# MeryylleA/Lunaris-Orion

Measured on AMD Instinct MI355X. Metric: 128x128 sprites/sec, VAE training step (train_hybrid.py _process_batch), latent_dim=512, higher is better.
Workload: dtype f16; 1 GPU; VAE-only training step (fwd+MSE/KL+bwd+clip+AdamW), per-GPU batch 64, latent_dim 512, teacher scalar 0 (--reward_scale 0 --quality_weight 0; the full hybrid step of BASELINE config 3 is the config3_full_hybrid object of a --full run at N=1), gradient_accumulation_steps 1, fp16 MFMA operands / fp32 accumulate, fp32 master weights; global_batch=64, latent_dim=512, parallelism=single, linear_weight_gradients=factored (never materialised)

## Files before the change

### lunaris_orion_amd/csrc/lo_conv.h

```cpp
#pragma once
#include "lo_common.h"

int lo_pack_weight(const float* w, f16* wp, const LoGeom& g, hipStream_t st);
int lo_pack_all(const LoPackJob* jobs_dev, int njobs, int nblocks, hipStream_t st, int block_base = 0);
int lo_pack_blocks(const LoGeom& g);
size_t lo_packed_weight_elems(const LoGeom& g);
static inline int lo_geom_packed_elems(const LoGeom& g) {
  int off = 0;
  for (int p = 0; p < g.n_phase; ++p) off += g.Cout * g.T[p] * g.Cin;
  return off;
}
static inline double lo_geom_flops(const LoGeom& g) {
  double f = 0;
  for (int p = 0; p < g.n_phase; ++p) f += 2.0 * g.B * g.GH * g.GW * (double)g.Cout * g.T[p] * g.Cin;
  return f;
}
static inline double lo_geom_bytes(const LoGeom& g) {
  return 2.0 * ((double)g.B * g.Hin * g.Win * g.Cin + (double)g.B * g.Hout * g.Wout * g.Cout + lo_geom_packed_elems(g));
}

struct LoGnBwdFuse {
  const f16* v; const float* stats; const float* gamma; const float* beta; float* P1;
  f16* dv = nullptr; float* P2 = nullptr; unsigned int* counter = nullptr; unsigned int target = 0; unsigned int* fail = nullptr;
  bool keep_out = false;
// ... 56 lines not shown
int lo_conv3_run(const LoGeom& g, const LoConvOp& op, const LoConvChoice& c, hipStream_t st);
int lo_convt4_patch_run(const LoGeom& g, const LoConvOp& op, const LoConvChoice& c, hipStream_t st);
int lo_convs2d_patch_run(const LoGeom& g, const LoConvOp& op, const LoConvChoice& c, hipStream_t st);
bool lo_conv3_pp_applies(const LoGeom& g);
bool lo_conv3_pp_f8_applies(const LoGeom& g);
int lo_conv3_pp_rows(const LoGeom& g);
int lo_conv3_run_pp_xf(const LoGeom& g, const f16* in, const f16* xc, const f16* kx, int nlev, const f16* wp, const float* bias,
                       f16* out, hipStream_t st, const LoConvExtra* ex);
int lo_conv3_run_pp_f8(const LoGeom& g, const uint8_t* in8, const uint8_t* w8, const float* wscale, const float* bias, f16* out,
                       hipStream_t st, const LoConvExtra* ex);

struct LoPackF8Job { const f16* src; uint8_t* dst; float* scale; int K[LO_MAX_PHASE]; int wofs[LO_MAX_PHASE]; int Cout, n_phase, block0; };
void lo_pack_f8_job(LoPackF8Job* j, const LoGeom& g, const f16* src, uint8_t* dst, float* scale, int block0);
int lo_pack_f8_all(const LoPackF8Job* jobs_dev, int njobs, int nblocks, hipStream_t st, int block_base = 0);
int lo_pack_f8_one(const LoGeom& g, const f16* wp, uint8_t* w8, float* wscale, hipStream_t st);
int lo_quantize_f8(const f16* x, uint8_t* x8, size_t n, hipStream_t st);

enum LoWgradKernel { LO_WK_WGRAD3 = 0, LO_WK_WGRAD2, LO_WK_TN };
enum LoWgradReduce { LO_WR_NONE = 0, LO_WR_ROWS, LO_WR_CONVT, LO_WR_SCATTER };
struct LoWgradChoice {
  int kernel;
  int bmw, bnw, bkp, stages;
  int taps;
  int tw;
  bool convt;
  int tiles;
  int units, units_per_split;
  int nsplit;
  int slabs;
  dim3 grid, block;
  bool direct;
  int reduce;
  dim3 rgrid, rblock;
};
LoWgradChoice lo_wgrad_choose(const LoGeom& g);
int lo_wgrad_run(const LoGeom& g, const f16* x, const f16* dy, float* slab, float* grad, float scale, hipStream_t st);
size_t lo_wgrad_slab_bytes(const LoGeom& g);
int lo_wgrad3_run(const LoGeom& g, const LoWgradChoice& p, const f16* x, const f16* dy, float* slab, hipStream_t st);
int lo_wgrad2_run(const LoGeom& g, const LoWgradChoice& p, const f16* x, const f16* dy, float* slab, hipStream_t st);
```

### lunaris_orion_amd/csrc/lo_norm.hip

```cpp
#include "lo_norm.h"
#include <stdlib.h>
#include <type_traits>

#define GN_EPS 1e-5f

enum { GN_MODE_PLAIN = 0, GN_MODE_SKIP = 1, GN_MODE_RES = 2 };

int lo_gn_nchunk(int HW, int C) {
  constexpr long chunk_elems = 16384;
  const long ce = (long)HW * C >= 524288 ? 2 * chunk_elems : chunk_elems;
  long e = (long)HW * C / ce;
  if (e < 1) e = 1;
  if (e > 256) e = 256;
  while (HW % e) --e;
  return (int)e;
}

struct GnFwdArgs {
  const f16* v;
  const float* partial;
  const float* gamma;
  const float* beta;
  const f16* other;
  f16* y;
// ... 399 lines not shown
  for (int c = tid; c < G; c += 256) {
    const int ccx = c >> 3, j = c & 7;
    float tot = 0.f;
    for (int sl = 0; sl < nslot; ++sl) tot += s_red[(sl * CG + ccx) * 8 + j];
    a.P2[(size_t)n * C + grp * G + c] = tot;
  }
}

__global__ __launch_bounds__(256) void lo_gn_param_finalize_kernel(const float* __restrict__ P1, const float* __restrict__ P2,
                                                                   float* dgamma, float* dbeta, float* dbias, int nblk, int C,
                                                                   float scale) {
  __shared__ float red[3][16][17];
  const int cl = threadIdx.x & 15, r = threadIdx.x >> 4;
  const int c = blockIdx.x * 16 + cl;
  float g1 = 0.f, g2 = 0.f, b = 0.f;
  if (c < C)
    for (int k = r; k < nblk; k += 16) {
      f32x2 p = *reinterpret_cast<const f32x2*>(P1 + ((size_t)k * C + c) * 2);
      g1 += p[0];
      g2 += p[1];
      b += P2[(size_t)k * C + c];
    }
  red[0][r][cl] = g1; red[1][r][cl] = g2; red[2][r][cl] = b;
  __syncthreads();
  if (r < 3 && c < C) {
    float tot = 0.f;
#pragma unroll
    for (int q = 0; q < 16; ++q) tot += red[r][q][cl];
    tot *= scale;
    if (r == 0) dbeta[c] = tot; else if (r == 1) dgamma[c] = tot; else dbias[c] = tot;
  }
}

__global__ __launch_bounds__(256) void lo_gn_finalize_all_kernel(LoGnFinJobs jobs, float scale) {
  __shared__ float red[3][64][5];
  int jb = 0;
  while (jb + 1 < jobs.n && (int)blockIdx.x >= jobs.j[jb + 1].block0) ++jb;
  const LoGnFinJob& J = jobs.j[jb];
  const int C = J.C;
  const int cl = threadIdx.x & 3, r = threadIdx.x >> 2;
  const int c = ((int)blockIdx.x - J.block0) * 4 + cl;
  float g1 = 0.f, g2 = 0.f, b = 0.f;
  if (c < C) {
    for (int k = r; k < J.nblk1; k += 64) {
      f32x2 p = *reinterpret_cast<const f32x2*>(J.P1 + ((size_t)k * C + c) * 2);
      g1 += p[0];
      g2 += p[1];
    }
    for (int k = r; k < J.nblk2; k += 64) b += J.P2[(size_t)k * C + c];
  }
  red[0][r][cl] = g1; red[1][r][cl] = g2; red[2][r][cl] = b;
  __syncthreads();
  if (threadIdx.x < 12) {
    const int which = threadIdx.x >> 2, c2 = threadIdx.x & 3;
    const int cg = ((int)blockIdx.x - J.block0) * 4 + c2;
    if (cg < C) {
      float tot = 0.f;
      for (int q = 0; q < 64; ++q) tot += red[which][q][c2];
      tot *= scale;
      if (which == 0) J.dbeta[cg] = tot; else if (which == 1) J.dgamma[cg] = tot; else J.dbias[cg] = tot;
    }
  }
}

__global__ __launch_bounds__(256) void lo_transpose_tile_kernel(const f16* __restrict__ src, f16* __restrict__ dst, uint8_t* __restrict__ dst8,
                                                                int R, int Cc) {
  __shared__ f16 tile[64][66];
  const int n = blockIdx.z, r0 = blockIdx.y * 64, c0 = blockIdx.x * 64;
  const f16* s = src + (size_t)n * R * Cc;
  const int tc = (threadIdx.x & 7) * 8, tr = threadIdx.x >> 3;
#pragma unroll
  for (int p = 0; p < 2; ++p) {
    const int r = tr + 32 * p;
    const f16x8 v = *reinterpret_cast<const f16x8*>(s + (size_t)(r0 + r) * Cc + c0 + tc);
#pragma unroll
    for (int j = 0; j < 8; ++j) tile[r][tc + j] = v[j];
  }
  __syncthreads();
  f16* d = dst + (size_t)n * R * Cc;
#pragma unroll
  for (int p = 0; p < 2; ++p) {
    const int c = tr + 32 * p;
    f16x8 v;
#pragma unroll
    for (int j = 0; j < 8; ++j) v[j] = tile[tc + j][c];
    const size_t off = (size_t)(c0 + c) * R + r0 + tc;
    *reinterpret_cast<f16x8*>(d + off) = v;
    if (dst8) {
// ... 175 lines not shown
    return LO_OK;
  }
  if (ch.form == LO_GNB_LOCAL) {
    LoProfScope _p(gn_layer_name("lo_gn_bwd_local", C, HW, mode), 0, 2.0 * B * HW * C * (mode == 2 ? 5 : 3), st);
    gn_launch_local(a, GnSlabSrc{nullptr, 0, nullptr, nullptr, 0}, B, st);
    LO_LAUNCH_CHECK("gn_bwd_local");
    return LO_OK;
  }
  LO_REQUIRE(C % 32 == 0 && C <= 512, "lo_gn_bwd: C=%d unsupported", C);
  if (ch.form == LO_GNB_TWO_PASS) {
    LoProfScope _p(gn_layer_name("lo_gn_bwd_reduce", C, HW, mode), 0, 2.0 * B * HW * C * (mode == 2 ? 4 : 2), st);
    gn_launch_reduce(a, B, st);
  }
  LO_LAUNCH_CHECK("gn_bwd_reduce");
  {
    LoProfScope _p(gn_layer_name("lo_gn_bwd_apply", C, HW, mode), 0, 2.0 * B * HW * C * (mode == 2 ? 4 : 3), st);
    gn_launch_apply(a, B, st);
  }
  LO_LAUNCH_CHECK("gn_bwd_apply");
  return LO_OK;
}

int lo_gn_bwd(const LoGnLayer& l, const LoGnBwd& op, float* dgamma, float* dbeta, float* dbias, float scale, hipStream_t st) {
  LoGnRows rows;
  int r = lo_gn_backward(l, op, st, &rows);
  if (r != LO_OK) return r;
  LoProfScope _p3("lo_gn_param_finalize", 0, 0, st);
  hipLaunchKernelGGL(lo_gn_param_finalize_kernel, dim3((l.C + 15) / 16), dim3(256), 0, st, op.P1, op.P2, dgamma, dbeta, dbias,
                     l.B * rows.p1, l.C, scale);
  LO_LAUNCH_CHECK("gn_param_finalize");
  return LO_OK;
}

int lo_gn_finalize_all(const LoGnFinJobs& jobs, float scale, hipStream_t st) {
  int nblocks = 0;
  for (int i = 0; i < jobs.n; ++i) nblocks += (jobs.j[i].C + 3) / 4;
  LoProfScope _p("lo_gn_finalize_all", 0, 0, st);
  hipLaunchKernelGGL(lo_gn_finalize_all_kernel, dim3(nblocks), dim3(256), 0, st, jobs, scale);
  LO_LAUNCH_CHECK("gn_finalize_all");
  return LO_OK;
}

int lo_nhwc_to_nchw_f16(const f16* src, f16* dst, int B, int HW, int C, hipStream_t st) {
  LO_REQUIRE(HW % 64 == 0 && C % 64 == 0, "lo_nhwc_to_nchw_f16: HW=%d, C=%d must be multiples of 64", HW, C);
  LoProfScope _p("lo_layout_transpose", 0, 4.0 * B * HW * C, st);
  LO_LAUNCH_STOP(lo_transpose_tile_kernel, dim3(C / 64, HW / 64, B), dim3(256), 0, st, src, dst, (uint8_t*)nullptr, HW, C);
  LO_LAUNCH_CHECK("nhwc_to_nchw");
  return LO_OK;
}
int lo_nchw_to_nhwc_f16(const f16* src, f16* dst, int B, int HW, int C, hipStream_t st, uint8_t* dst8) {
  LO_REQUIRE(HW % 64 == 0 && C % 64 == 0, "lo_nchw_to_nhwc_f16: HW=%d, C=%d must be multiples of 64", HW, C);
  LoProfScope _p("lo_layout_transpose", 0, 4.0 * B * HW * C, st);
  LO_LAUNCH_STOP(lo_transpose_tile_kernel, dim3(HW / 64, C / 64, B), dim3(256), 0, st, src, dst, dst8, C, HW);
  LO_LAUNCH_CHECK("nchw_to_nhwc");
  return LO_OK;
}

template <typename TI, typename TO>
__global__ __launch_bounds__(256) void lo_transpose_convert_kernel(const TI* __restrict__ src, TO* __restrict__ dst, int R, int Cc, float scale) {
  __shared__ float tile[64][65];
  const int n = blockIdx.z, r0 = blockIdx.y * 64, c0 = blockIdx.x * 64;
  const TI* s = src + (size_t)n * R * Cc;
  const int tc = threadIdx.x & 63, tr = threadIdx.x >> 6;
#pragma unroll
  for (int p = 0; p < 16; ++p) tile[tr + 4 * p][tc] = (float)s[(size_t)(r0 + tr + 4 * p) * Cc + c0 + tc] * scale;
  __syncthreads();
  TO* d = dst + (size_t)n * R * Cc;
#pragma unroll
  for (int p = 0; p < 16; ++p) d[(size_t)(c0 + tr + 4 * p) * R + r0 + tc] = (TO)tile[tc][tr + 4 * p];
// ... 14 lines not shown
```

### lunaris_orion_amd/csrc/lo_vae_plan.hip

```cpp
#include "lo_vae.h"
#include <memory>

namespace {
struct Arena {
  size_t off = 0;
  size_t take(size_t bytes) {
    size_t o = off;
    off += (bytes + 255) & ~(size_t)255;
    return o;
  }
};
bool env_is_zero(const char* v) { return v && atoi(v) == 0; }
const int kEncCh[5] = {3, 64, 128, 256, 512};
const int kDecCh[5] = {512, 256, 128, 64, 32};
}

static bool layer_takes_f8(const LoGeom& gf) {
  if (lo_conv_choose(gf, {.bias = true, .gn_partial = true, .f8 = true}).kernel == LO_CK_NONE) return false;
  return lo_conv_choose(gf, {.bias = true, .gn_partial = true}).kernel != LO_CK_CONVT4_PATCH;
}

static int setup_conv_layer(ConvLayer& c, int kind, int B, int H, int W, int Cin, int Cout, int p_w, Arena& ar, bool first, bool fp8_fwd) {
  c.kind = kind; c.H = H; c.W = W; c.Cin = Cin; c.Cout = Cout;
  c.p_w = p_w; c.p_b = p_w + 1; c.p_gw = p_w + 2; c.p_gb = p_w + 3;
// ... 292 lines not shown
  const float sc = h->fac.scale / (float)world;
  LO_TRY(lo_lowrank_materialize_gathered(G + h->p_off[h->idx_fc_mu_w], vae_fac_in_block(h, base, h->o_fac_xT), vae_fac_in_block(h, base, h->o_fac_dmlT),
                                         blk, world, 2 * L, 32768, h->B, sc, st));
  return lo_lowrank_materialize_gathered(G + h->p_off[h->idx_dfc_w], vae_fac_in_block(h, base, h->o_fac_zT), vae_fac_in_block(h, base, h->o_fac_gfcT),
                                         blk, world, 32768, L, h->B, sc, st);
}
extern "C" int lo_vae_linear_factored(const LoVae* h) { return h ? vae_flat_lacks_linear(h) : 0; }
extern "C" int lo_vae_num_params(const LoVae* h) { return h->nparam; }
extern "C" size_t lo_vae_param_offset(const LoVae* h, int i) { return (i >= 0 && i < h->nparam) ? h->p_off[i] : (size_t)-1; }
extern "C" size_t lo_vae_param_numel(const LoVae* h, int i) { return (i >= 0 && i < h->nparam) ? h->p_numel[i] : 0; }
extern "C" size_t lo_vae_flat_elems(const LoVae* h) { return h->flat_elems; }
extern "C" size_t lo_vae_workspace_bytes(const LoVae* h) { return h->ws_bytes; }

extern "C" int lo_vae_debug_tensor(const LoVae* h, int which, int s, int k, size_t* byte_offset, int* dims4) {
  LO_REQUIRE(h && byte_offset && dims4 && s >= 0 && s < 4 && k >= 0 && k < 3, "lo_vae_debug_tensor: bad argument");
  const ConvLayer* c = which == 0 ? &h->enc[s][k] : ((which == 1 || which == 3) ? &h->dec[s] : (which == 2 ? &h->enc[s][2] : nullptr));
  LO_REQUIRE(c, "lo_vae_debug_tensor: unknown tensor kind %d", which);
  *byte_offset = which == 2 ? h->o_eout[s] : (which == 3 ? c->o_a : c->o_v);
  dims4[0] = h->B; dims4[1] = c->Ho; dims4[2] = c->Wo; dims4[3] = c->Cout;
  return LO_OK;
}

extern "C" int lo_vae_debug_tensor_ex(const LoVae* h, int which, int s, int k, size_t* byte_offset, int* dims4, int* elem_bytes) {
  LO_REQUIRE(h && byte_offset && dims4 && elem_bytes && s >= 0 && s < 4 && k >= 0 && k < 3, "lo_vae_debug_tensor_ex: bad argument");
  *elem_bytes = 2;
  if (which >= 0 && which <= 3) return lo_vae_debug_tensor(h, which, s, k, byte_offset, dims4);
  dims4[0] = h->B;
  if (which == 9) { *byte_offset = h->o_h0; dims4[1] = dims4[2] = 8; dims4[3] = 512; return LO_OK; }
  if (which == 10) {
    LO_REQUIRE(s < 3, "lo_vae_debug_tensor_ex: three skip gradients, asked for %d", s);
    *byte_offset = h->o_skipg[s]; dims4[1] = dims4[2] = 64 >> s; dims4[3] = 64 << s;
    return LO_OK;
  }
  LO_REQUIRE(which >= 4 && which <= 8 && !(which == 4 && k == 2), "lo_vae_debug_tensor_ex: unknown tensor kind %d (k = %d)", which, k);
  const ConvLayer* c = (which == 6 || which == 8) ? &h->dec[s] : &h->enc[s][k];
  if (which == 5 || which == 6) {
    *byte_offset = c->o_stats; *elem_bytes = 4;
    dims4[1] = 8; dims4[2] = 2; dims4[3] = 1;
    return LO_OK;
  }
  *byte_offset = which == 4 ? c->o_a : ((c == &h->enc[0][0] && !c->dv_done) ? h->o_G[3] : c->o_dv);
  dims4[1] = c->Ho; dims4[2] = c->Wo; dims4[3] = c->Cout;
  return LO_OK;
}
extern "C" int lo_vae_layer_plan(const LoVae* h, int dec, int s, int k, int* info4) {
  LO_REQUIRE(h && info4 && s >= 0 && s < 4 && k >= 0 && k < 3, "lo_vae_layer_plan: bad argument");
  const ConvLayer& c = dec ? h->dec[s] : h->enc[s][k];
  info4[0] = c.f8 ? 1 : 0; info4[1] = c.MT; info4[2] = c.sk_fwd; info4[3] = c.sk_dgrad;
  return LO_OK;
}

extern "C" int lo_vae_sync_fail_word(const LoVae* h, size_t* byte_offset, int* fused_layers) {
  LO_REQUIRE(h && byte_offset, "lo_vae_sync_fail_word: null argument");
  *byte_offset = h->o_sync_fail;
  if (fused_layers) {
    int n = 0;
    for_each_layer(h, [&](const ConvLayer& c) { n += c.gnf ? 1 : 0; });
    *fused_layers = n;
  }
  return LO_OK;
}

extern "C" int lo_vae_set_async_handover(LoVae* h, int on) {
  LO_REQUIRE(h, "lo_vae_set_async_handover: null handle");
  h->async_handover = on != 0;
  return LO_OK;
// ... 70 lines not shown
```

### lunaris_orion_amd/csrc/lo_wgrad.hip

```cpp
#include "lo_conv.h"
#include "lo_conv_dev.h"
#include <stdarg.h>
#include <stdio.h>
#include <string.h>
#include <stdlib.h>

struct WgradArgs {
  const f16* x;
  const f16* dy;
  float* slab;
  float* grad;
  float scale;
  int direct;
  int taps;
  int M;
  int nsplit;
  int msteps_per_split;
  int packed_elems;
  LoGeom g;
};

template <int BMW, int BNW, int NSTAGE, int BKP>
__global__ __launch_bounds__(256) void lo_wgrad_tn(WgradArgs a) {
  static_assert(BKP == 32 || BKP == 64, "pixels per K step");
// ... 194 lines not shown
                                                                   int total, int nsplit, float scale) {
  __shared__ float part[4][9][64];
  __shared__ int tap_of_rs[9];
  const int x = threadIdx.x, t = threadIdx.y, sg = threadIdx.z, G = blockDim.z;
  const int cblocks = g.Cin >> 6;
  const int n = blockIdx.x / cblocks, c0 = (blockIdx.x - n * cblocks) << 6;
  if (sg == 0 && x == 0) tap_of_rs[g.rs[0][t]] = t;
  const size_t i = (size_t)n * 9 * g.Cin + (size_t)t * g.Cin + c0 + 4 * x;
  const float* src = slab + i;
  f32x4 v = {0.f, 0.f, 0.f, 0.f};
  int s = sg;
  for (; s + 3 * G < nsplit; s += 4 * G) {
    f32x4 a0 = *reinterpret_cast<const f32x4*>(src + (size_t)s * total);
    f32x4 a1 = *reinterpret_cast<const f32x4*>(src + (size_t)(s + G) * total);
    f32x4 a2 = *reinterpret_cast<const f32x4*>(src + (size_t)(s + 2 * G) * total);
    f32x4 a3 = *reinterpret_cast<const f32x4*>(src + (size_t)(s + 3 * G) * total);
    v += a0; v += a1; v += a2; v += a3;
  }
  for (; s < nsplit; s += G) v += *reinterpret_cast<const f32x4*>(src + (size_t)s * total);
  *reinterpret_cast<f32x4*>(&part[sg][t][4 * x]) = v;
  __syncthreads();
  const int w = x + 16 * (t + 9 * sg);
  if (w >= 144) return;
  f32x4 o;
#pragma unroll
  for (int e = 0; e < 4; ++e) {
    const int f = 4 * w + e, cc = f / 9, rs = f - cc * 9, tt = tap_of_rs[rs];
    float acc = part[0][tt][cc];
    for (int q = 1; q < G; ++q) acc += part[q][tt][cc];
    o[e] = acc * scale;
  }
  *reinterpret_cast<f32x4*>(grad + (size_t)n * g.sn + (size_t)c0 * 9 + 4 * w) = o;
}
__global__ __launch_bounds__(256) void lo_wgrad_reduce_convt_kernel(const float* __restrict__ slab, float* __restrict__ grad, LoGeom g,
                                                                    int total, int nsplit, float scale) {
  __shared__ float outb[16][4][16];
  const int tid = threadIdx.x, x = tid & 3, seg = tid >> 2, nl = seg >> 4, p = (seg >> 2) & 3, t = seg & 3;
  const int cblocks = g.Cin >> 4;
  const int nb = blockIdx.x / cblocks, c0 = (blockIdx.x - nb * cblocks) << 4, n0 = nb << 2;
  const size_t i = (size_t)g.wofs[p] + (size_t)(n0 + nl) * 4 * g.Cin + (size_t)t * g.Cin + c0 + 4 * x;
  const float* src = slab + i;
  f32x4 v = {0.f, 0.f, 0.f, 0.f};
  int s = 0;
  for (; s + 4 <= nsplit; s += 4) {
    f32x4 a0 = *reinterpret_cast<const f32x4*>(src + (size_t)s * total);
    f32x4 a1 = *reinterpret_cast<const f32x4*>(src + (size_t)(s + 1) * total);
    f32x4 a2 = *reinterpret_cast<const f32x4*>(src + (size_t)(s + 2) * total);
    f32x4 a3 = *reinterpret_cast<const f32x4*>(src + (size_t)(s + 3) * total);
    v += a0; v += a1; v += a2; v += a3;
  }
  for (; s < nsplit; ++s) v += *reinterpret_cast<const f32x4*>(src + (size_t)s * total);
  const int rs = g.rs[p][t];
#pragma unroll
  for (int e = 0; e < 4; ++e) outb[4 * x + e][nl][rs] = v[e] * scale;
  __syncthreads();
  const int cc = tid >> 4, q = tid & 15;
  *reinterpret_cast<f32x4*>(grad + (size_t)(c0 + cc) * g.sc + (size_t)n0 * 16 + 4 * q) =
      *reinterpret_cast<const f32x4*>(&outb[cc][q >> 2][(q & 3) * 4]);
}
static bool lo_wgrad_reduce_convt_applies(const LoGeom& g) {
  if (g.n_phase != 4 || g.sn != 16 || g.sc != g.Cout * 16 || g.Cin % 16 != 0 || g.Cout % 4 != 0) return false;
  for (int p = 0; p < 4; ++p)
    if (g.T[p] != 4 || g.wofs[p] != p * 4 * g.Cin * g.Cout) return false;
  return true;
}
static bool lo_wgrad_reduce_rows_applies(const LoGeom& g) {
  return g.n_phase == 1 && g.T[0] == 9 && g.sc == 9 && g.sn == 9 * g.Cin && g.wofs[0] == 0 && g.Cin % 64 == 0;
}

static bool wgrad3_applies(const LoGeom& g) {
  if (g.n_phase != 1 || g.T[0] != 9 || g.in_stride != 1 || g.out_stride != 1) return false;
  if (g.Cin % 64 || g.Cout % 64 || g.Hin != g.Hout || g.Win != g.Wout) return false;
  if (g.Win % 16 == 0) return g.Hin % 2 == 0;
  return g.Win == 8 && g.Hin % 4 == 0;
}
struct Wgrad2Shape { bool convt; int Hc, Wc, Ca, Cf; };
static bool wgrad2_applies(const LoGeom& g, Wgrad2Shape* s) {
  const bool s2 = g.n_phase == 1 && g.T[0] == 9 && g.in_stride == 2 && g.out_stride == 1;
  const bool ct = g.n_phase == 4 && g.in_stride == 1 && g.out_stride == 2 && g.T[0] == 4 && g.T[3] == 4;
  if (!s2 && !ct) return false;
  *s = {ct, s2 ? g.Hout : g.Hin, s2 ? g.Wout : g.Win, s2 ? g.Cout : g.Cin, s2 ? g.Cin : g.Cout};
  return s->Hc % 4 == 0 && s->Wc % 8 == 0 && s->Ca % 64 == 0 && (s->Cf % 64 == 0 || s->Cf == 32);
}
static bool lo_wgrad_s2_enabled() {
  static const bool on = [] { const char* e = getenv("LO_WGRAD_S2"); return !(e && atoi(e) == 0); }();
  return on;
}

struct WgradPolicy { int target, floor, min_units, max_splits; };
// ... 25 lines not shown
    c.kernel = LO_WK_WGRAD2;
    c.convt = s2.convt;
    c.tiles = (s2.Ca / 64) * ((s2.Cf + 63) / 64);
    c.units = g.B * s2.Hc * s2.Wc / 32;
    c.block = dim3(512);
  } else {
    c.kernel = LO_WK_TN;
    pol = &kPolicyTn;
    const long M = (long)g.B * g.GH * g.GW;
    c.bmw = g.Cout % 128 == 0 ? 128 : 64;
    c.bnw = g.Cin % 128 == 0 ? 128 : 64;
    c.bkp = M % 64 == 0 && M >= 1024 ? 64 : 32;
    c.stages = c.bkp == 64 && c.bmw + c.bnw > 192 ? 2 : 3;
    for (int p = 0; p < g.n_phase; ++p) c.taps += g.T[p];
    c.tiles = ((g.Cout + c.bmw - 1) / c.bmw) * (g.Cin / c.bnw) * c.taps;
    c.units = (int)((M + c.bkp - 1) / c.bkp);
    c.block = dim3(256);
  }
  const int total = lo_geom_packed_elems(g);
  const int want = wgrad_wanted_splits(c.tiles, c.units, (long)total * 4, *pol);
  c.units_per_split = (c.units + want - 1) / want;
  c.nsplit = (c.units + c.units_per_split - 1) / c.units_per_split;
  c.slabs = c.kernel == LO_WK_WGRAD2 ? c.nsplit : want;
  c.grid = dim3(c.tiles * c.nsplit);
  c.direct = c.kernel == LO_WK_TN && c.nsplit == 1 && g.sc == 1;
  if (c.direct) {
    c.reduce = LO_WR_NONE;
  } else if (lo_wgrad_reduce_rows_applies(g)) {
    c.reduce = LO_WR_ROWS;
    c.rgrid = dim3(g.Cout * (g.Cin / 64));
    c.rblock = dim3(16, 9, c.nsplit >= 4 ? 4 : c.nsplit);
  } else if (lo_wgrad_reduce_convt_applies(g)) {
    c.reduce = LO_WR_CONVT;
    c.rgrid = dim3((g.Cout / 4) * (g.Cin / 16));
    c.rblock = dim3(256);
  } else {
    c.reduce = LO_WR_SCATTER;
    c.rgrid = dim3((total / 4 + 63) / 64);
    c.rblock = dim3(256);
  }
  return c;
}

size_t lo_wgrad_slab_bytes(const LoGeom& g) { return (size_t)lo_wgrad_choose(g).slabs * lo_geom_packed_elems(g) * sizeof(float); }

static int wgrad_tn_run(const LoGeom& g, const LoWgradChoice& p, const f16* x, const f16* dy, float* slab, float* grad, float scale, hipStream_t st) {
  LO_REQUIRE(g.Cin % 64 == 0 && g.Cout % 32 == 0, "lo_wgrad_run: need Cin %% 64 == 0 and Cout %% 32 == 0 (Cin=%d Cout=%d)", g.Cin, g.Cout);
  LO_REQUIRE(g.lg_hin >= 0 && g.lg_win >= 0 && g.lg_cin >= 0 && g.lg_hout >= 0 && g.lg_wout >= 0,
             "lo_wgrad_run: tensor dims must be powers of two");
  WgradArgs a;
  a.x = x; a.dy = dy; a.slab = slab; a.g = g; a.grad = grad; a.scale = scale;
  a.M = g.B * g.GH * g.GW;
  a.packed_elems = lo_geom_packed_elems(g);
  a.taps = p.taps; a.nsplit = p.nsplit; a.msteps_per_split = p.units_per_split;
  a.direct = p.direct ? 1 : 0;
#define LO_WG(BMW, BNW)                                                                                                          \
  do {                                                                                                                           \
    if (p.bkp == 64 && p.stages == 3) hipLaunchKernelGGL((lo_wgrad_tn<BMW, BNW, 3, 64>), p.grid, p.block, 0, st, a);             \
    else if (p.bkp == 64) hipLaunchKernelGGL((lo_wgrad_tn<BMW, BNW, 2, 64>), p.grid, p.block, 0, st, a);                         \
    else hipLaunchKernelGGL((lo_wgrad_tn<BMW, BNW, 3, 32>), p.grid, p.block, 0, st, a);                                          \
  } while (0)
  if (p.bmw == 128 && p.bnw == 128) LO_WG(128, 128);
  else if (p.bmw == 128 && p.bnw == 64) LO_WG(128, 64);
  else if (p.bmw == 64 && p.bnw == 128) LO_WG(64, 128);
  else LO_WG(64, 64);
#undef LO_WG
  LO_LAUNCH_CHECK("wgrad_tn");
  return LO_OK;
}

static int lo_wgrad_reduce_launch(const LoGeom& g, const LoWgradChoice& p, const float* slab, float* grad, float scale, hipStream_t st) {
  auto* const kernel = p.reduce == LO_WR_ROWS ? lo_wgrad_reduce_rows_kernel : p.reduce == LO_WR_CONVT ? lo_wgrad_reduce_convt_kernel : lo_wgrad_reduce_kernel;
  hipLaunchKernelGGL(kernel, p.rgrid, p.rblock, 0, st, slab, grad, g, lo_geom_packed_elems(g), p.nsplit, scale);
  LO_LAUNCH_CHECK("wgrad_reduce");
  return LO_OK;
}

int lo_wgrad_run(const LoGeom& g, const f16* x, const f16* dy, float* slab, float* grad, float scale, hipStream_t st) {
  static const char* const scope[3] = {"lo_wgrad3x3_mt", "lo_wgrad_s2_mt", "lo_wgrad_tn"};
  const LoWgradChoice p = lo_wgrad_choose(g);
  {
    LoProfScope _p(lo_prof_geom_name(scope[p.kernel], g), lo_geom_flops(g), lo_geom_bytes(g), st);
    int r = p.kernel == LO_WK_WGRAD3   ? lo_wgrad3_run(g, p, x, dy, slab, st)
            : p.kernel == LO_WK_WGRAD2 ? lo_wgrad2_run(g, p, x, dy, slab, st)
                                       : wgrad_tn_run(g, p, x, dy, slab, grad, scale, st);
    if (r != LO_OK) return r;
  }
  if (p.reduce == LO_WR_NONE) return LO_OK;
  LoProfScope _p2(lo_prof_geom_name("lo_wgrad_reduce", g), 0, 4.0 * lo_geom_packed_elems(g) * (p.nsplit + 1), st);
  return lo_wgrad_reduce_launch(g, p, slab, grad, scale, st);
}
```

### lunaris_orion_amd/csrc/lo_wgrad2.hip

```cpp
#include "lo_conv.h"
#include "lo_conv_dev.h"

struct Wgrad2Args {
  const f16* a;
  const f16* f;
  float* slab;
  int B, Hc, Wc, Ca, Cf;
  int nsplit, chunks_per_split, nchunks;
  int packed_elems;
  int Cin;
  int wofs[4];
};

template <bool CONVT>
__global__ __launch_bounds__(512) void lo_wgrad_s2_mt(Wgrad2Args a) {
  constexpr int R = CONVT ? 4 : 3, NTAP = R * R;
  constexpr int TH = 4, TW = 8;
  constexpr int PH = 2 * TH + R - 1, PWH = 10;
  constexpr int PROWS = PH * 2 * PWH;
  constexpr int PQ = (PROWS + 7) / 8;
  static_assert(4 + PQ <= 32, "eight waves x four instructions per chunk");
  constexpr int A_BYTES = 32 * 128, P_BYTES = PQ * 1024;
  constexpr int STAGE = A_BYTES + P_BYTES;
  constexpr int NSTAGE = 3, D = 2;
  constexpr int NTW = (NTAP + 1) / 2;
  __shared__ __attribute__((aligned(1024))) unsigned char smem[NSTAGE * STAGE + 1024];

  const int tid = threadIdx.x, lane = tid & 63;
  const int wave = __builtin_amdgcn_readfirstlane(tid >> 6);
  const int wa = wave & 1, wf = (wave >> 1) & 1, wt = wave >> 2;
  const int tiles_f = (a.Cf + 63) >> 6, tiles = (a.Ca >> 6) * tiles_f;
  const int wid = lo_xcd_remap(blockIdx.x, gridDim.x);
  const int tile = wid % tiles, split = wid / tiles;
  const int a0 = (tile / tiles_f) * 64, f0 = (tile % tiles_f) * 64;
  const int q_begin = split * a.chunks_per_split;
  const int q_end = min(a.nchunks, q_begin + a.chunks_per_split);
  const int nq = q_end - q_begin;
  const int chunks_x = a.Wc / TW, chunks_img = chunks_x * (a.Hc / TH);
  const int Hf = 2 * a.Hc, Wf = 2 * a.Wc;
  const f16* zpage = reinterpret_cast<const f16*>(lo_zero_page);

  int s_kind[4], s_off[4], s_py[4], s_px[4];
  unsigned int s_lds[4];
#pragma unroll
  for (int j = 0; j < 4; ++j) {
    const int q = wave * 4 + j;
    const int row8 = lane >> 3, pos = lane & 7;
    if (q < 4) {
      const int arow = q * 8 + row8;
      s_kind[j] = 0;
      s_py[j] = arow / TW; s_px[j] = arow % TW;
      s_off[j] = (s_py[j] * a.Wc + s_px[j]) * a.Ca + a0 + ((((pos >> 1) ^ lo_tr_swz<128>(arow)) << 1) | (pos & 1)) * 8;
      s_lds[j] = (unsigned int)(q * 1024);
    } else if (q - 4 < PQ) {
      const int prow = (q - 4) * 8 + row8;
      const int py = prow / (2 * PWH), rem = prow - py * (2 * PWH), par = rem / PWH, hx = rem - par * PWH;
      const int px = 2 * hx + par;
      const int ch = f0 + ((((pos >> 1) ^ lo_tr_swz<128>(prow)) << 1) | (pos & 1)) * 8;
      const bool ok = prow < PROWS && px < 2 * TW + R - 1 && ch < a.Cf;
      s_kind[j] = ok ? 1 : 2;
      s_py[j] = py - 1; s_px[j] = px - 1;
      s_off[j] = ((py - 1) * Wf + (px - 1)) * a.Cf + ch;
      s_lds[j] = (unsigned int)(A_BYTES + (q - 4) * 1024);
// ... 40 lines not shown
#pragma unroll
    for (int h = 0; h < 2; ++h) {
      const int Rr = trow + 16 * h, blk = wa * 2 + mi;
      aoff[mi][h] = Rr * 128 + ((blk ^ lo_tr_swz<128>(Rr)) * 32) + tsub;
    }
  int boff[NTW][2];
#pragma unroll
  for (int tt = 0; tt < NTW; ++tt)
#pragma unroll
    for (int h = 0; h < 2; ++h) {
      const int t = wt * NTW + tt;
      const int tq = t < NTAP ? t : 0;
      const int r = tq / R, s = tq % R;
      const int kk = trow + 16 * h, ky = kk / TW, kx = kk % TW;
      const int prow = ((2 * ky + r) * 2 + (s & 1)) * PWH + kx + (s >> 1);
      boff[tt][h] = A_BYTES + prow * 128 + (((wf * 2) ^ lo_tr_swz<128>(prow)) * 32) + tsub;
    }

  f32x4 acc[NTW][2][2];
#pragma unroll
  for (int tt = 0; tt < NTW; ++tt)
#pragma unroll
    for (int mi = 0; mi < 2; ++mi)
#pragma unroll
      for (int ni = 0; ni < 2; ++ni) acc[tt][mi][ni] = (f32x4){0.f, 0.f, 0.f, 0.f};

  auto tr = [&](const unsigned char* p) __attribute__((always_inline)) {
    return __builtin_amdgcn_ds_read_tr16_b64_v4f16((h16x4 __attribute__((address_space(3)))*)p);
  };
  auto frag = [&](const unsigned char* lo_p, const unsigned char* hi_p) __attribute__((always_inline)) {
    h16x4 lo = tr(lo_p), hi = tr(hi_p);
    return (f16x8){(f16)lo[0], (f16)lo[1], (f16)lo[2], (f16)lo[3], (f16)hi[0], (f16)hi[1], (f16)hi[2], (f16)hi[3]};
  };
  const bool f_live = f0 + wf * 32 < a.Cf;

  if (nq > 0) {
#pragma unroll
    for (int s = 0; s < D; ++s) issue(s);
    int rs = 0, ws = D % NSTAGE;
    for (int it = 0; it < nq; ++it) {
      LO_VMCNT(4 * (D - 1));
      __builtin_amdgcn_s_barrier();
      issue(ws);
      if (f_live) {
        const unsigned char* sbase = smem + rs * STAGE;
        f16x8 af[2];
#pragma unroll
        for (int mi = 0; mi < 2; ++mi) af[mi] = frag(sbase + aoff[mi][0], sbase + aoff[mi][1]);
#pragma unroll
        for (int tt = 0; tt < NTW; ++tt) {
          if (NTAP % 2 == 0 || tt + 1 < NTW || wt == 0) {
            f16x8 bf[2];
#pragma unroll
            for (int ni = 0; ni < 2; ++ni) bf[ni] = frag(sbase + (boff[tt][0] ^ (ni * 32)), sbase + (boff[tt][1] ^ (ni * 32)));
#pragma unroll
            for (int mi = 0; mi < 2; ++mi)
#pragma unroll
              for (int ni = 0; ni < 2; ++ni)
                acc[tt][mi][ni] = __builtin_amdgcn_mfma_f32_16x16x32_f16(af[mi], bf[ni], acc[tt][mi][ni], 0, 0, 0);
          }
        }
      }
      rs = (rs + 1 == NSTAGE) ? 0 : rs + 1;
      ws = (ws + 1 == NSTAGE) ? 0 : ws + 1;
    }
    LO_VMCNT(0);
  }
  if (!f_live) return;
  float* slab = a.slab + (size_t)split * a.packed_elems;
#pragma unroll
  for (int tt = 0; tt < NTW; ++tt) {
    const int t = wt * NTW + tt;
    if (t >= NTAP) continue;
    const int r = t / R, s = t % R;
#pragma unroll
    for (int mi = 0; mi < 2; ++mi)
#pragma unroll
      for (int ni = 0; ni < 2; ++ni) {
        const int cf = f0 + wf * 32 + ni * 16 + (lane & 15);
#pragma unroll
        for (int j = 0; j < 4; ++j) {
          const int ca = a0 + wa * 32 + mi * 16 + (lane >> 4) * 4 + j;
          size_t idx;
          if (CONVT) {
            const int p = ((r & 1) ? 0 : 2) + ((s & 1) ? 0 : 1), tp = (r >> 1) * 2 + (s >> 1);
            idx = (size_t)a.wofs[p] + (size_t)cf * (4 * a.Cin) + tp * a.Cin + ca;
          } else {
            idx = (size_t)ca * (9 * a.Cin) + t * a.Cin + cf;
          }
          if (cf < a.Cf) slab[idx] = acc[tt][mi][ni][j];
        }
      }
  }
}

int lo_wgrad2_run(const LoGeom& g, const LoWgradChoice& p, const f16* x, const f16* dy, float* slab, hipStream_t st) {
  LO_REQUIRE(p.kernel == LO_WK_WGRAD2, "lo_wgrad2_run: the plan names another weight-gradient kernel");
  const bool s2 = !p.convt;
  Wgrad2Args a;
  a.a = s2 ? dy : x; a.f = s2 ? x : dy; a.slab = slab;
  a.B = g.B; a.Hc = s2 ? g.Hout : g.Hin; a.Wc = s2 ? g.Wout : g.Win;
  a.Ca = s2 ? g.Cout : g.Cin; a.Cf = s2 ? g.Cin : g.Cout;
  a.nchunks = p.units; a.nsplit = p.nsplit; a.chunks_per_split = p.units_per_split;
  a.packed_elems = lo_geom_packed_elems(g);
  a.Cin = g.Cin;
  for (int q = 0; q < 4; ++q) a.wofs[q] = q < g.n_phase ? g.wofs[q] : 0;
  if (s2) hipLaunchKernelGGL((lo_wgrad_s2_mt<false>), p.grid, p.block, 0, st, a);
  else hipLaunchKernelGGL((lo_wgrad_s2_mt<true>), p.grid, p.block, 0, st, a);
  LO_LAUNCH_CHECK("wgrad_s2_mt");
  return LO_OK;
}
```

Measured before the change: 24760 sprites/s.

## Widen GN finalize vectorization, add fine-grained convT wgrad reduce, narrow-Cf wgrad wave split

The GroupNorm finalize kernel now handles 16 channels per block with f32x4 loads and a 4-deep unrolled accumulation, which cuts the block count and widens the memory accesses. The transposed-conv weight-gradient slab reduce gains a fine-grained variant (scalar lanes, one n per block) used when the coarse grid would have fewer than 512 blocks, to raise parallelism. The s2 wgrad MFMA kernel gains a NARROW mode for Cf==32 that splits taps across 4 waves instead of leaving half the waves idle on dead f-columns. A debug tensor accessor for P1/P2 is also added. The finalize now requires C to be a multiple of 4 and recomputes each job's block0.

```diff
diff --git a/lunaris_orion_amd/csrc/lo_conv.h b/lunaris_orion_amd/csrc/lo_conv.h
--- a/lunaris_orion_amd/csrc/lo_conv.h
+++ b/lunaris_orion_amd/csrc/lo_conv.h
@@ -112,6 +112,7 @@
   bool direct;
   int reduce;
   dim3 rgrid, rblock;
+  bool rfine;
 };
 LoWgradChoice lo_wgrad_choose(const LoGeom& g);
 int lo_wgrad_run(const LoGeom& g, const f16* x, const f16* dy, float* slab, float* grad, float scale, hipStream_t st);
diff --git a/lunaris_orion_amd/csrc/lo_norm.hip b/lunaris_orion_amd/csrc/lo_norm.hip
--- a/lunaris_orion_amd/csrc/lo_norm.hip
+++ b/lunaris_orion_amd/csrc/lo_norm.hip
@@ -455,28 +455,56 @@
   }
 }
 
+#define LO_GN_FIN_CH 16
 __global__ __launch_bounds__(256) void lo_gn_finalize_all_kernel(LoGnFinJobs jobs, float scale) {
-  __shared__ float red[3][64][5];
+  __shared__ float red[3][64][LO_GN_FIN_CH + 1];
   int jb = 0;
   while (jb + 1 < jobs.n && (int)blockIdx.x >= jobs.j[jb + 1].block0) ++jb;
   const LoGnFinJob& J = jobs.j[jb];
   const int C = J.C;
-  const int cl = threadIdx.x & 3, r = threadIdx.x >> 2;
-  const int c = ((int)blockIdx.x - J.block0) * 4 + cl;
-  float g1 = 0.f, g2 = 0.f, b = 0.f;
+  const int cq = threadIdx.x & 3, r = threadIdx.x >> 2;
+  const int cb = ((int)blockIdx.x - J.block0) * LO_GN_FIN_CH, c = cb + cq * 4;
+  f32x4 pa = {0.f, 0.f, 0.f, 0.f}, pb = {0.f, 0.f, 0.f, 0.f};
+  f32x4 b = {0.f, 0.f, 0.f, 0.f};
   if (c < C) {
-    for (int k = r; k < J.nblk1; k += 64) {
-      f32x2 p = *reinterpret_cast<const f32x2*>(J.P1 + ((size_t)k * C + c) * 2);
-      g1 += p[0];
-      g2 += p[1];
-    }
-    for (int k = r; k < J.nblk2; k += 64) b += J.P2[(size_t)k * C + c];
-  }
-  red[0][r][cl] = g1; red[1][r][cl] = g2; red[2][r][cl] = b;
-  __syncthreads();
-  if (threadIdx.x < 12) {
-    const int which = threadIdx.x >> 2, c2 = threadIdx.x & 3;
-    const int cg = ((int)blockIdx.x - J.block0) * 4 + c2;
+    const float* p1 = J.P1 + (size_t)c * 2;
+    const float* p2 = J.P2 + c;
+    const size_t s1 = (size_t)C * 2, s2 = (size_t)C;
+    int k = r;
+    for (; k + 192 < J.nblk1; k += 256) {
+      f32x4 xa[4], xb[4];
+#pragma unroll
+      for (int j = 0; j < 4; ++j) {
+        xa[j] = *reinterpret_cast<const f32x4*>(p1 + (size_t)(k + 64 * j) * s1);
+        xb[j] = *reinterpret_cast<const f32x4*>(p1 + (size_t)(k + 64 * j) * s1 + 4);
+      }
+#pragma unroll
+      for (int j = 0; j < 4; ++j) { pa += xa[j]; pb += xb[j]; }
+    }
+    for (; k < J.nblk1; k += 64) {
+      pa += *reinterpret_cast<const f32x4*>(p1 + (size_t)k * s1);
+      pb += *reinterpret_cast<const f32x4*>(p1 + (size_t)k * s1 + 4);
+    }
+    k = r;
+    for (; k + 192 < J.nblk2; k += 256) {
+      f32x4 x[4];
+#pragma unroll
+      for (int j = 0; j < 4; ++j) x[j] = *reinterpret_cast<const f32x4*>(p2 + (size_t)(k + 64 * j) * s2);
+#pragma unroll
+      for (int j = 0; j < 4; ++j) b += x[j];
+    }
+    for (; k < J.nblk2; k += 64) b += *reinterpret_cast<const f32x4*>(p2 + (size_t)k * s2);
+  }
+  float* r0 = &red[0][r][cq * 4];
+  float* r1 = &red[1][r][cq * 4];
+  float* r2 = &red[2][r][cq * 4];
+  r0[0] = pa[0]; r0[1] = pa[2]; r0[2] = pb[0]; r0[3] = pb[2];
+  r1[0] = pa[1]; r1[1] = pa[3]; r1[2] = pb[1]; r1[3] = pb[3];
+  r2[0] = b[0]; r2[1] = b[1]; r2[2] = b[2]; r2[3] = b[3];
+  __syncthreads();
+  if (threadIdx.x < 3 * LO_GN_FIN_CH) {
+    const int which = threadIdx.x / LO_GN_FIN_CH, c2 = threadIdx.x % LO_GN_FIN_CH;
+    const int cg = cb + c2;
     if (cg < C) {
       float tot = 0.f;
       for (int q = 0; q < 64; ++q) tot += red[which][q][c2];
@@ -718,9 +746,14 @@
   return LO_OK;
 }
 
-int lo_gn_finalize_all(const LoGnFinJobs& jobs, float scale, hipStream_t st) {
+int lo_gn_finalize_all(const LoGnFinJobs& jobs_in, float scale, hipStream_t st) {
+  LoGnFinJobs jobs = jobs_in;
   int nblocks = 0;
-  for (int i = 0; i < jobs.n; ++i) nblocks += (jobs.j[i].C + 3) / 4;
+  for (int i = 0; i < jobs.n; ++i) {
+    LO_REQUIRE(jobs.j[i].C % 4 == 0, "lo_gn_finalize_all: C = %d is no multiple of 4", jobs.j[i].C);
+    jobs.j[i].block0 = nblocks;
+    nblocks += (jobs.j[i].C + LO_GN_FIN_CH - 1) / LO_GN_FIN_CH;
+  }
   LoProfScope _p("lo_gn_finalize_all", 0, 0, st);
   hipLaunchKernelGGL(lo_gn_finalize_all_kernel, dim3(nblocks), dim3(256), 0, st, jobs, scale);
   LO_LAUNCH_CHECK("gn_finalize_all");
diff --git a/lunaris_orion_amd/csrc/lo_vae_plan.hip b/lunaris_orion_amd/csrc/lo_vae_plan.hip
--- a/lunaris_orion_amd/csrc/lo_vae_plan.hip
+++ b/lunaris_orion_amd/csrc/lo_vae_plan.hip
@@ -348,6 +348,14 @@
     *byte_offset = h->o_skipg[s]; dims4[1] = dims4[2] = 64 >> s; dims4[3] = 64 << s;
     return LO_OK;
   }
+  if (which >= 11 && which <= 14) {
+    const ConvLayer* c = which >= 13 ? &h->dec[s] : &h->enc[s][k];
+    const bool p1 = which == 11 || which == 13;
+    LO_REQUIRE(c->np1 > 0 && c->np2 > 0, "lo_vae_debug_tensor_ex: no backward has left P1 / P2 rows for this layer");
+    *byte_offset = p1 ? c->o_P1 : c->o_P2; *elem_bytes = 4;
+    dims4[1] = p1 ? c->np1 : c->np2; dims4[2] = c->Cout; dims4[3] = p1 ? 2 : 1;
+    return LO_OK;
+  }
   LO_REQUIRE(which >= 4 && which <= 8 && !(which == 4 && k == 2), "lo_vae_debug_tensor_ex: unknown tensor kind %d (k = %d)", which, k);
   const ConvLayer* c = (which == 6 || which == 8) ? &h->dec[s] : &h->enc[s][k];
   if (which == 5 || which == 6) {
diff --git a/lunaris_orion_amd/csrc/lo_wgrad.hip b/lunaris_orion_amd/csrc/lo_wgrad.hip
--- a/lunaris_orion_amd/csrc/lo_wgrad.hip
+++ b/lunaris_orion_amd/csrc/lo_wgrad.hip
@@ -250,29 +250,36 @@
   }
   *reinterpret_cast<f32x4*>(grad + (size_t)n * g.sn + (size_t)c0 * 9 + 4 * w) = o;
 }
+template <int NB, typename V>
+__device__ __forceinline__ void lo_slab_sum(V& v, const float* __restrict__ src, int s, int nsplit, int step, size_t total) {
+  for (; s + (NB - 1) * step < nsplit; s += NB * step) {
+    V a[NB];
+#pragma unroll
+    for (int j = 0; j < NB; ++j) a[j] = *reinterpret_cast<const V*>(src + (size_t)(s + j * step) * total);
+#pragma unroll
+    for (int j = 0; j < NB; ++j) v += a[j];
+  }
+  if constexpr (NB > 1) lo_slab_sum<NB / 2>(v, src, s, nsplit, step, total);
+}
+template <int VW, int NN>
 __global__ __launch_bounds__(256) void lo_wgrad_reduce_convt_kernel(const float* __restrict__ slab, float* __restrict__ grad, LoGeom g,
                                                                     int total, int nsplit, float scale) {
-  __shared__ float outb[16][4][16];
-  const int tid = threadIdx.x, x = tid & 3, seg = tid >> 2, nl = seg >> 4, p = (seg >> 2) & 3, t = seg & 3;
+  constexpr int XW = 16 / VW;
+  static_assert(XW * NN * 16 == 256, "thread = (column of the 16 channels, n, phase, tap)");
+  typedef float vec __attribute__((ext_vector_type(VW)));
+  __shared__ float outb[16][NN][16];
+  const int tid = threadIdx.x, x = tid % XW, seg = tid / XW, nl = seg >> 4, p = (seg >> 2) & 3, t = seg & 3;
   const int cblocks = g.Cin >> 4;
-  const int nb = blockIdx.x / cblocks, c0 = (blockIdx.x - nb * cblocks) << 4, n0 = nb << 2;
-  const size_t i = (size_t)g.wofs[p] + (size_t)(n0 + nl) * 4 * g.Cin + (size_t)t * g.Cin + c0 + 4 * x;
-  const float* src = slab + i;
-  f32x4 v = {0.f, 0.f, 0.f, 0.f};
-  int s = 0;
-  for (; s + 4 <= nsplit; s += 4) {
-    f32x4 a0 = *reinterpret_cast<const f32x4*>(src + (size_t)s * total);
-    f32x4 a1 = *reinterpret_cast<const f32x4*>(src + (size_t)(s + 1) * total);
-    f32x4 a2 = *reinterpret_cast<const f32x4*>(src + (size_t)(s + 2) * total);
-    f32x4 a3 = *reinterpret_cast<const f32x4*>(src + (size_t)(s + 3) * total);
-    v += a0; v += a1; v += a2; v += a3;
-  }
-  for (; s < nsplit; ++s) v += *reinterpret_cast<const f32x4*>(src + (size_t)s * total);
+  const int nb = blockIdx.x / cblocks, c0 = (blockIdx.x - nb * cblocks) << 4, n0 = nb * NN;
+  const size_t i = (size_t)g.wofs[p] + (size_t)(n0 + nl) * 4 * g.Cin + (size_t)t * g.Cin + c0 + VW * x;
+  vec v = 0.f;
+  lo_slab_sum<VW == 1 ? 16 : 4>(v, slab + i, 0, nsplit, 1, (size_t)total);
   const int rs = g.rs[p][t];
 #pragma unroll
-  for (int e = 0; e < 4; ++e) outb[4 * x + e][nl][rs] = v[e] * scale;
+  for (int e = 0; e < VW; ++e) outb[VW * x + e][nl][rs] = v[e] * scale;
   __syncthreads();
-  const int cc = tid >> 4, q = tid & 15;
+  if (tid >= 64 * NN) return;
+  const int cc = tid / (4 * NN), q = tid % (4 * NN);
   *reinterpret_cast<f32x4*>(grad + (size_t)(c0 + cc) * g.sc + (size_t)n0 * 16 + 4 * q) =
       *reinterpret_cast<const f32x4*>(&outb[cc][q >> 2][(q & 3) * 4]);
 }
@@ -364,7 +371,8 @@
     c.rblock = dim3(16, 9, c.nsplit >= 4 ? 4 : c.nsplit);
   } else if (lo_wgrad_reduce_convt_applies(g)) {
     c.reduce = LO_WR_CONVT;
-    c.rgrid = dim3((g.Cout / 4) * (g.Cin / 16));
+    c.rfine = (g.Cout / 4) * (g.Cin / 16) < 512;
+    c.rgrid = dim3((c.rfine ? g.Cout : g.Cout / 4) * (g.Cin / 16));
     c.rblock = dim3(256);
   } else {
     c.reduce = LO_WR_SCATTER;
@@ -402,7 +410,10 @@
 }
 
 static int lo_wgrad_reduce_launch(const LoGeom& g, const LoWgradChoice& p, const float* slab, float* grad, float scale, hipStream_t st) {
-  auto* const kernel = p.reduce == LO_WR_ROWS ? lo_wgrad_reduce_rows_kernel : p.reduce == LO_WR_CONVT ? lo_wgrad_reduce_convt_kernel : lo_wgrad_reduce_kernel;
+  auto* const kernel = p.reduce == LO_WR_ROWS    ? lo_wgrad_reduce_rows_kernel
+                       : p.reduce != LO_WR_CONVT ? lo_wgrad_reduce_kernel
+                       : p.rfine                 ? lo_wgrad_reduce_convt_kernel<1, 1>
+                                                 : lo_wgrad_reduce_convt_kernel<4, 4>;
   hipLaunchKernelGGL(kernel, p.rgrid, p.rblock, 0, st, slab, grad, g, lo_geom_packed_elems(g), p.nsplit, scale);
   LO_LAUNCH_CHECK("wgrad_reduce");
   return LO_OK;
diff --git a/lunaris_orion_amd/csrc/lo_wgrad2.hip b/lunaris_orion_amd/csrc/lo_wgrad2.hip
--- a/lunaris_orion_amd/csrc/lo_wgrad2.hip
+++ b/lunaris_orion_amd/csrc/lo_wgrad2.hip
@@ -12,8 +12,9 @@
   int wofs[4];
 };
 
-template <bool CONVT>
+template <bool CONVT, bool NARROW>
 __global__ __launch_bounds__(512) void lo_wgrad_s2_mt(Wgrad2Args a) {
+  static_assert(CONVT || !NARROW, "the 32-channel decode exists for the transposed form only");
   constexpr int R = CONVT ? 4 : 3, NTAP = R * R;
   constexpr int TH = 4, TW = 8;
   constexpr int PH = 2 * TH + R - 1, PWH = 10;
@@ -23,12 +24,13 @@
   constexpr int A_BYTES = 32 * 128, P_BYTES = PQ * 1024;
   constexpr int STAGE = A_BYTES + P_BYTES;
   constexpr int NSTAGE = 3, D = 2;
-  constexpr int NTW = (NTAP + 1) / 2;
+  constexpr int NWT = NARROW ? 4 : 2;
+  constexpr int NTW = (NTAP + NWT - 1) / NWT;
   __shared__ __attribute__((aligned(1024))) unsigned char smem[NSTAGE * STAGE + 1024];
 
   const int tid = threadIdx.x, lane = tid & 63;
   const int wave = __builtin_amdgcn_readfirstlane(tid >> 6);
-  const int wa = wave & 1, wf = (wave >> 1) & 1, wt = wave >> 2;
+  const int wa = wave & 1, wf = NARROW ? 0 : (wave >> 1) & 1, wt = NARROW ? wave >> 1 : wave >> 2;
   const int tiles_f = (a.Cf + 63) >> 6, tiles = (a.Ca >> 6) * tiles_f;
   const int wid = lo_xcd_remap(blockIdx.x, gridDim.x);
   const int tile = wid % tiles, split = wid / tiles;
@@ -135,7 +137,7 @@
     h16x4 lo = tr(lo_p), hi = tr(hi_p);
     return (f16x8){(f16)lo[0], (f16)lo[1], (f16)lo[2], (f16)lo[3], (f16)hi[0], (f16)hi[1], (f16)hi[2], (f16)hi[3]};
   };
-  const bool f_live = f0 + wf * 32 < a.Cf;
+  const bool f_live = NARROW || f0 + wf * 32 < a.Cf;
 
   if (nq > 0) {
 #pragma unroll
@@ -152,7 +154,7 @@
         for (int mi = 0; mi < 2; ++mi) af[mi] = frag(sbase + aoff[mi][0], sbase + aoff[mi][1]);
 #pragma unroll
         for (int tt = 0; tt < NTW; ++tt) {
-          if (NTAP % 2 == 0 || tt + 1 < NTW || wt == 0) {
+          if (NTAP % NWT == 0 || tt + 1 < NTW || wt == 0) {
             f16x8 bf[2];
 #pragma unroll
             for (int ni = 0; ni < 2; ++ni) bf[ni] = frag(sbase + (boff[tt][0] ^ (ni * 32)), sbase + (boff[tt][1] ^ (ni * 32)));
@@ -208,8 +210,9 @@
   a.packed_elems = lo_geom_packed_elems(g);
   a.Cin = g.Cin;
   for (int q = 0; q < 4; ++q) a.wofs[q] = q < g.n_phase ? g.wofs[q] : 0;
-  if (s2) hipLaunchKernelGGL((lo_wgrad_s2_mt<false>), p.grid, p.block, 0, st, a);
-  else hipLaunchKernelGGL((lo_wgrad_s2_mt<true>), p.grid, p.block, 0, st, a);
+  if (s2) hipLaunchKernelGGL((lo_wgrad_s2_mt<false, false>), p.grid, p.block, 0, st, a);
+  else if (a.Cf == 32) hipLaunchKernelGGL((lo_wgrad_s2_mt<true, true>), p.grid, p.block, 0, st, a);
+  else hipLaunchKernelGGL((lo_wgrad_s2_mt<true, false>), p.grid, p.block, 0, st, a);
   LO_LAUNCH_CHECK("wgrad_s2_mt");
   return LO_OK;
 }
```

Result: no change. 24920 sprites/s, median of 6 (+0.7%).
